# OnurBasci/TransformerBasedNavierStokeSolver

Hardware: AMD Instinct MI355X
Metric: ns64_train_samples_per_s (higher is better)
Workload: dtype f32

## Files before the change

### transformerbasednavierstokesolver_amd/csrc/pa2d_conv_halo.hip

```cpp
#include "pa2d_gemm_common.h"

namespace {
constexpr int TH = 8, TW = 32, BM = TH * TW, BN = 128;
constexpr int HH = TH + 2, HWD = TW + 2, HROWS = HH * HWD;
}

template <int NT, typename TO = float, int TPB = (NT == 1 ? 3 : 1), bool MF16 = false>
__global__ __launch_bounds__(512, 1) void conv_halo_kernel(const KCParams p, const int tiles_x, const int tiles_y,
                                                           const int nimg) {
    constexpr int PITCHB = NT * 64 + (MF16 ? 32 : 16);
    constexpr int PIECES = NT * 4;
    constexpr int A_BYTES = HROWS * PITCHB;
    constexpr int B_TAP = BN * PITCHB;
    constexpr int B_STAGE = TPB * B_TAP;
    constexpr int SPC = 9 / TPB;
    constexpr int AP_IT = (HROWS * PIECES + 255) / 256;
    constexpr int BP_IT = (TPB * BN * PIECES) / 256;
    constexpr int TM = 4, TN = 2;
    static_assert(9 % TPB == 0, "taps per stage");
    extern __shared__ __attribute__((aligned(16))) unsigned char smem[];
    unsigned char* const a_s = smem;
    unsigned char* const b_s = smem + A_BYTES;

    const int tid = threadIdx.x, lane = tid & 63, wave = tid >> 6;
    const int tiles_n = (p.N + BN - 1) / BN;
    const int tiles_m = nimg * tiles_y * tiles_x;
    const int tmx = (tiles_m + 7) / 8;
    const int xcd = blockIdx.x & 7, slot = blockIdx.x >> 3;
    const int tile_m = xcd * tmx + slot / tiles_n;
    const int tile_n = slot % tiles_n;
    if (tile_m >= tiles_m || slot / tiles_n >= tmx) return;
    const int img = tile_m / (tiles_y * tiles_x);
    const int trem = tile_m - img * (tiles_y * tiles_x);
    const int y0 = (trem / tiles_x) * TH, x0 = (trem % tiles_x) * TW;
    const int nch = p.Cin / 32;
    const int nk = nch * 9;
    const int nst = nch * SPC;

    if (wave >= 4) {
        const int ptid = tid - 256;
        const __amdgpu_buffer_rsrc_t ra_rsrc = make_rsrc(p.A, p.a_bytes);
        const __amdgpu_buffer_rsrc_t rb_rsrc = make_rsrc(p.B, p.b_bytes);
        unsigned ap_off[AP_IT], ap_lds[AP_IT];
#pragma unroll
        for (int s = 0; s < AP_IT; ++s) {
            const int q = ptid + 256 * s, row = q / PIECES, piece = q - row * PIECES;
            const int hy = row / HWD, hx = row - hy * HWD;
            const int yy = y0 - 1 + hy, xx = x0 - 1 + hx;
            const bool ok = row < HROWS && (unsigned)yy < (unsigned)p.H && (unsigned)xx < (unsigned)p.W;
            ap_off[s] = ok ? ((unsigned)((img * p.H + yy) * p.W + xx) * (unsigned)(nch * PIECES) + piece) * 16u : OOB_OFF;
            ap_lds[s] = row < HROWS ? (unsigned)(row * PITCHB + piece * 16) : 0xFFFFFFFFu;
        }
        unsigned bp_off[BP_IT], bp_lds[BP_IT];
#pragma unroll
        for (int s = 0; s < BP_IT; ++s) {
            const int q = ptid + 256 * s, tapi = q / (BN * PIECES), r = q - tapi * (BN * PIECES);
            const int row = r / PIECES, piece = r - row * PIECES;
            const int gn = tile_n * BN + row;
            bp_off[s] = gn < p.N ? ((unsigned)gn * (unsigned)nk * PIECES + (unsigned)(tapi * PIECES) + piece) * 16u : OOB_OFF;
            bp_lds[s] = tapi * B_TAP + row * PITCHB + piece * 16;
        }
        u32x4 rq[AP_IT], rp0[BP_IT], rp1[BP_IT];
#define HA_LOAD(chunk_)                                                                                    \
    {                                                                                                      \
        const unsigned sh_ = (unsigned)(chunk_) * (PIECES * 16u);                                          \
        _Pragma("unroll") for (int s = 0; s < AP_IT; ++s)                                                  \
            rq[s] = __builtin_amdgcn_raw_buffer_load_b128(ra_rsrc, ap_off[s] != OOB_OFF ? ap_off[s] + sh_ : OOB_OFF, 0, 0); \
    }
#define HA_STORE()                                                                                         \
    {                                                                                                      \
        _Pragma("unroll") for (int s = 0; s < AP_IT; ++s)                                                  \
            if (ap_lds[s] != 0xFFFFFFFFu) *reinterpret_cast<u32x4*>(a_s + ap_lds[s]) = rq[s];              \
    }
#define HB_LOAD(sg_, RP)                       \
    {                                                                                                      \
        _Pragma("unroll") for (int s = 0; s < BP_IT; ++s)                                                  \
            RP[s] = __builtin_amdgcn_raw_buffer_load_b128(                                                 \
                rb_rsrc, bp_off[s] != OOB_OFF ? bp_off[s] + (unsigned)((sg_) * TPB) * (PIECES * 16u) : OOB_OFF, 0, 0); \
    }
#define HB_STORE(stage_, RP)                                                                               \
    {                                                                                                      \
        _Pragma("unroll") for (int s = 0; s < BP_IT; ++s)                                                  \
            *reinterpret_cast<u32x4*>(b_s + (stage_) * B_STAGE + bp_lds[s]) = RP[s];                       \
    }
#define HB_STEP(sg_, RP_NEXT)                      \
    {                                                                                                      \
        if ((sg_) + 1 < nst) {                                                                             \
            HB_STORE(((sg_) + 1) & 1, RP_NEXT)                                                             \
            if ((sg_) + 5 < nst) HB_LOAD((sg_) + 5, RP_NEXT)                                               \
        }                                                                                                  \
        __syncthreads();                                                              \
        if ((sg_) % SPC == SPC - 1 && (sg_) + 1 < nst) {   \
            HA_STORE()                                                                                     \
            if ((sg_) / SPC + 2 < nch) HA_LOAD((sg_) / SPC + 2)                                            \
            __syncthreads();                                                                               \
        }                                                                                                  \
    }
        u32x4 rp2[BP_IT], rp3[BP_IT];
        HA_LOAD(0)
        HB_LOAD(0, rp0)
        if (nst > 1) HB_LOAD(1, rp1)
        if (nst > 2) HB_LOAD(2, rp2)
        if (nst > 3) HB_LOAD(3, rp3)
        HA_STORE()
        HB_STORE(0, rp0)
        if (nch > 1) HA_LOAD(1)
        if (nst > 4) HB_LOAD(4, rp0)
        __syncthreads();
        for (int sg = 0; sg < nst; sg += 4) {
            HB_STEP(sg, rp1)
            if (sg + 1 < nst) HB_STEP(sg + 1, rp2)
            if (sg + 2 < nst) HB_STEP(sg + 2, rp3)
            if (sg + 3 < nst) HB_STEP(sg + 3, rp0)
        }
#undef HB_STEP
#undef HA_LOAD
#undef HA_STORE
#undef HB_LOAD
#undef HB_STORE
        return;
    }

    const int wm = wave >> 1, wn = wave & 1;
    if constexpr (MF16) {
        static_assert(NT == 3 && TPB == 1, "the 16x16x32 consumers are written for the split engine");
        const int li = lane & 15, kq = lane >> 4;
        f32x4 acc[8][4];
#pragma unroll
        for (int ib = 0; ib < 8; ++ib)
#pragma unroll
            for (int j = 0; j < 4; ++j) acc[ib][j] = f32x4{0.f, 0.f, 0.f, 0.f};
        const unsigned a_frag = (unsigned)((((wm * 4 + 1) * HWD) + 1 + li) * PITCHB + kq * 16);
        const unsigned b_frag = (unsigned)((wn * 64 + li) * PITCHB + kq * 16);
        __syncthreads();
        int tap = 0;
        for (int sg = 0; sg < nst; ++sg) {
            const int dy = tap / 3 - 1, dx = tap - (tap / 3) * 3 - 1;
            const unsigned char* af_base = a_s + a_frag + (dy * HWD + dx) * PITCHB;
            const unsigned char* bf_base = b_s + (sg & 1) * B_STAGE + b_frag;
            bf16x8 bf[4][NT];
#pragma unroll
            for (int j = 0; j < 4; ++j)
#pragma unroll
                for (int q = 0; q < NT; ++q) bf[j][q] = *reinterpret_cast<const bf16x8*>(bf_base + j * 16 * PITCHB + q * 64);
#pragma unroll
            for (int ib = 0; ib < 8; ++ib) {
                bf16x8 af[NT];
#pragma unroll
                for (int q = 0; q < NT; ++q)
                    af[q] = *reinterpret_cast<const bf16x8*>(af_base + (ib >> 1) * (HWD * PITCHB) + (ib & 1) * 16 * PITCHB + q * 64);
#pragma unroll
                for (int j = 0; j < 4; ++j) {
                    acc[ib][j] = __builtin_amdgcn_mfma_f32_16x16x32_bf16(bf[j][1], af[1], acc[ib][j], 0, 0, 0);
                    acc[ib][j] = __builtin_amdgcn_mfma_f32_16x16x32_bf16(bf[j][0], af[2], acc[ib][j], 0, 0, 0);
                    acc[ib][j] = __builtin_amdgcn_mfma_f32_16x16x32_bf16(bf[j][2], af[0], acc[ib][j], 0, 0, 0);
                    acc[ib][j] = __builtin_amdgcn_mfma_f32_16x16x32_bf16(bf[j][0], af[1], acc[ib][j], 0, 0, 0);
                    acc[ib][j] = __builtin_amdgcn_mfma_f32_16x16x32_bf16(bf[j][1], af[0], acc[ib][j], 0, 0, 0);
                    acc[ib][j] = __builtin_amdgcn_mfma_f32_16x16x32_bf16(bf[j][0], af[0], acc[ib][j], 0, 0, 0);
                }
            }
            ++tap;
            __syncthreads();
            if (tap == 9) {
                tap = 0;
                if (sg + 1 < nst) __syncthreads();
            }
        }
        const __amdgpu_buffer_rsrc_t rc = make_rsrc(p.C, p.c_bytes);
        constexpr unsigned ES = Act<TO>::ES;
        const unsigned ldc_b = (unsigned)p.ldc * ES, roww_b = (unsigned)p.W * ldc_b;
        const bool inside = y0 + TH <= p.H && x0 + TW <= p.W;
#pragma unroll
        for (int j = 0; j < 4; ++j) {
            const int col = tile_n * BN + wn * 64 + j * 16 + 4 * kq;
            const bool col_ok = col < p.N;
            float bv[4];
#pragma unroll
            for (int e = 0; e < 4; ++e)
                bv[e] = (p.bias && col_ok) ? (col + e < p.bias_split ? p.bias[col + e] : p.bias2[col + e - p.bias_split]) : 0.f;
#pragma unroll
            for (int ib = 0; ib < 8; ++ib) {
                const int y = y0 + wm * 4 + (ib >> 1), x = x0 + (ib & 1) * 16 + li;
                const bool ok = col_ok && (inside || (y < p.H && x < p.W));
                const unsigned off = ok ? (unsigned)((img * p.H + y) * p.W + x) * ldc_b + (unsigned)col * ES : OOB_OFF;
                float v[4];
#pragma unroll
                for (int e = 0; e < 4; ++e) v[e] = acc[ib][j][e] + bv[e];
                if constexpr (ES == 4) {
                    const u32x4 u = {__float_as_uint(v[0]), __float_as_uint(v[1]), __float_as_uint(v[2]), __float_as_uint(v[3])};
                    __builtin_amdgcn_raw_buffer_store_b128(u, rc, off, 0, 0);
                } else {
                    typedef unsigned int u32x2_ __attribute__((ext_vector_type(2)));
                    const u32x2_ u = {(unsigned)f32_to_bf16_bits(v[0]) | ((unsigned)f32_to_bf16_bits(v[1]) << 16),
                                      (unsigned)f32_to_bf16_bits(v[2]) | ((unsigned)f32_to_bf16_bits(v[3]) << 16)};
                    __builtin_amdgcn_raw_buffer_store_b64(u, rc, off, 0, 0);
                }
            }
        }
        (void)roww_b;
        return;
    }
    f32x16 acc[TM][TN];
#pragma unroll
    for (int i = 0; i < TM; ++i)
#pragma unroll
        for (int j = 0; j < TN; ++j)
#pragma unroll
            for (int r = 0; r < 16; ++r) acc[i][j][r] = 0.f;
    const unsigned a_frag = (unsigned)((((wm * 4 + 1) * HWD) + 1 + (lane & 31)) * PITCHB + (lane >> 5) * 16);
    const unsigned b_frag = (unsigned)((wn * 64 + (lane & 31)) * PITCHB + (lane >> 5) * 16);
    __syncthreads();
    int tap = 0;
    for (int sg = 0; sg < nst; ++sg) {
#pragma unroll
        for (int tt = 0; tt < TPB; ++tt, ++tap) {
            const int dy = tap / 3 - 1, dx = tap - (tap / 3) * 3 - 1;
            const unsigned char* af_base = a_s + a_frag + (dy * HWD + dx) * PITCHB;
            const unsigned char* bf_base = b_s + (sg & 1) * B_STAGE + tt * B_TAP + b_frag;
#pragma unroll
            for (int ks = 0; ks < 2; ++ks) {
                bf16x8 af[TM][NT], bf[TN][NT];
#pragma unroll
                for (int i = 0; i < TM; ++i)
#pragma unroll
                    for (int q = 0; q < NT; ++q)
                        af[i][q] = *reinterpret_cast<const bf16x8*>(af_base + i * (HWD * PITCHB) + q * 64 + ks * 32);
#pragma unroll
                for (int j = 0; j < TN; ++j)
#pragma unroll
                    for (int q = 0; q < NT; ++q)
                        bf[j][q] = *reinterpret_cast<const bf16x8*>(bf_base + j * 32 * PITCHB + q * 64 + ks * 32);
#pragma unroll
                for (int i = 0; i < TM; ++i)
#pragma unroll
                    for (int j = 0; j < TN; ++j) {
                        if constexpr (NT == 3) {
                            acc[i][j] = __builtin_amdgcn_mfma_f32_32x32x16_bf16(af[i][1], bf[j][1], acc[i][j], 0, 0, 0);
                            acc[i][j] = __builtin_amdgcn_mfma_f32_32x32x16_bf16(af[i][2], bf[j][0], acc[i][j], 0, 0, 0);
                            acc[i][j] = __builtin_amdgcn_mfma_f32_32x32x16_bf16(af[i][0], bf[j][2], acc[i][j], 0, 0, 0);
                            acc[i][j] = __builtin_amdgcn_mfma_f32_32x32x16_bf16(af[i][1], bf[j][0], acc[i][j], 0, 0, 0);
                            acc[i][j] = __builtin_amdgcn_mfma_f32_32x32x16_bf16(af[i][0], bf[j][1], acc[i][j], 0, 0, 0);
                        }
                        acc[i][j] = __builtin_amdgcn_mfma_f32_32x32x16_bf16(af[i][0], bf[j][0], acc[i][j], 0, 0, 0);
                    }
            }
        }
        __syncthreads();
        if (tap == 9) {
            tap = 0;
            if (sg + 1 < nst) __syncthreads();
        }
    }

    const __amdgpu_buffer_rsrc_t rc = make_rsrc(p.C, p.c_bytes);
    constexpr unsigned ES = Act<TO>::ES;
    if (y0 + TH <= p.H && x0 + TW <= p.W) {
        const unsigned ldc_b = (unsigned)p.ldc * ES, roww_b = (unsigned)p.W * ldc_b;
#pragma unroll
        for (int j = 0; j < TN; ++j) {
            const int col = tile_n * BN + wn * 64 + j * 32 + (lane & 31);
            const bool col_ok = col < p.N;
            const float bv = (p.bias && col_ok) ? (col < p.bias_split ? p.bias[col] : p.bias2[col - p.bias_split]) : 0.f;
            const unsigned vo = col_ok ? (unsigned)((img * p.H + y0 + wm * 4) * p.W + x0 + 4 * (lane >> 5)) * ldc_b + (unsigned)col * ES
                                       : OOB_OFF;
#pragma unroll
            for (int i = 0; i < TM; ++i)
#pragma unroll
                for (int r = 0; r < 16; ++r) {
                    const unsigned so = (unsigned)i * roww_b + (unsigned)((r & 3) + 8 * (r >> 2)) * ldc_b;
                    if constexpr (ES == 4) __builtin_amdgcn_raw_buffer_store_b32(__float_as_uint(acc[i][j][r] + bv), rc, vo, so, 0);
                    else __builtin_amdgcn_raw_buffer_store_b16(f32_to_bf16_bits(acc[i][j][r] + bv), rc, vo, so, 0);
                }
        }
        return;
    }
#pragma unroll
    for (int j = 0; j < TN; ++j) {
        const int col = tile_n * BN + wn * 64 + j * 32 + (lane & 31);
        const bool col_ok = col < p.N;
        const float bv = (p.bias && col_ok) ? (col < p.bias_split ? p.bias[col] : p.bias2[col - p.bias_split]) : 0.f;
#pragma unroll
        for (int i = 0; i < TM; ++i) {
            const int y = y0 + wm * 4 + i;
            const unsigned rowbase = (unsigned)((img * p.H + y) * p.W);
#pragma unroll
            for (int r = 0; r < 16; ++r) {
                const int x = x0 + 4 * (lane >> 5) + (r & 3) + 8 * (r >> 2);
                const bool ok = col_ok && y < p.H && x < p.W;
                Act<TO>::bst1(rc, ok ? ((rowbase + (unsigned)x) * (unsigned)p.ldc + (unsigned)col) * ES : OOB_OFF,
                              acc[i][j][r] + bv);
            }
        }
    }
}

static int halo_policy() { return pa2d_env().conv_halo; }

bool conv_halo_applies(const KCParams& p) {
    const int pol = halo_policy();
    if (p.taps == 27) return false;
    if (pol == 0 || !p.apre || (p.Cin % 32) != 0 || p.H <= 0 || p.W <= 0 || (p.M % (p.H * p.W)) != 0) return false;
    const long long tiles = (long long)(p.M / (p.H * p.W)) * ceil_div(p.H, TH) * ceil_div(p.W, TW) * ceil_div(p.N, BN);
    return pol == 2 || tiles >= 512;
}

int launch_conv_halo(const KCParams& p, hipStream_t st) {
    const int NT = p.engine == 2 ? 1 : 3;
    const int tiles_x = ceil_div(p.W, TW), tiles_y = ceil_div(p.H, TH), nimg = p.M / (p.H * p.W);
    const int tiles_m = nimg * tiles_y * tiles_x, tiles_n = ceil_div(p.N, BN);
    const dim3 grid(ceil_div(tiles_m, 8) * 8 * tiles_n);
    const int pitch = NT * 64 + 16;
    const int smem = HROWS * pitch + 2 * (NT == 1 ? 3 : 1) * BN * pitch;
    if (NT == 3 && pa2d_env().conv_mfma16 && (p.N % 4) == 0 && (p.ldc % 4) == 0) {
        const int smem16 = (HROWS + 2 * BN) * (3 * 64 + 32);
        {
            hipError_t e = hipFuncSetAttribute(reinterpret_cast<const void*>(&conv_halo_kernel<3, float, 1, true>),
                                               hipFuncAttributeMaxDynamicSharedMemorySize, smem16);
            if (e != hipSuccess) return (int)e;
        }
        hipLaunchKernelGGL((conv_halo_kernel<3, float, 1, true>), grid, dim3(512), smem16, st, p, tiles_x, tiles_y, nimg);
    } else if (NT == 3) {
        {
            hipError_t e = hipFuncSetAttribute(reinterpret_cast<const void*>(&conv_halo_kernel<3>),
                                               hipFuncAttributeMaxDynamicSharedMemorySize, smem);
            if (e != hipSuccess) return (int)e;
        }
        hipLaunchKernelGGL((conv_halo_kernel<3>), grid, dim3(512), smem, st, p, tiles_x, tiles_y, nimg);
    } else if (p.io_bf16) {
        {
            hipError_t e = hipFuncSetAttribute(reinterpret_cast<const void*>(&conv_halo_kernel<1, bf16_t>),
                                               hipFuncAttributeMaxDynamicSharedMemorySize, smem);
            if (e != hipSuccess) return (int)e;
        }
        hipLaunchKernelGGL((conv_halo_kernel<1, bf16_t>), grid, dim3(512), smem, st, p, tiles_x, tiles_y, nimg);
    } else {
        {
            hipError_t e = hipFuncSetAttribute(reinterpret_cast<const void*>(&conv_halo_kernel<1>),
                                               hipFuncAttributeMaxDynamicSharedMemorySize, smem);
            if (e != hipSuccess) return (int)e;
        }
        hipLaunchKernelGGL((conv_halo_kernel<1>), grid, dim3(512), smem, st, p, tiles_x, tiles_y, nimg);
    }
    PA2D_CHECK_LAUNCH();
    return PA2D_OK;
}
```

### transformerbasednavierstokesolver_amd/csrc/pa2d_gemm.hip

```cpp
#include "pa2d_gemm_common.h"
#include <string.h>


static Pa2dEnv read_env() {
    auto is = [](const char* n, const char* pre) { const char* e = getenv(n); return e && strncmp(e, pre, strlen(pre)) == 0; };
    auto num = [](const char* n, int dflt) { const char* e = getenv(n); return (e && e[0]) ? atoi(e) : dflt; };
    Pa2dEnv v;
    v.conv_halo = is("PA2D_CONV_HALO", "o") ? 0 : (is("PA2D_CONV_HALO", "f") ? 2 : 1);
    v.mc_big_off = is("PA2D_MC_BIG", "o") ? 1 : 0;
    v.kc_bk16 = num("PA2D_KC_BK", 0) == 16 ? 1 : 0;
    v.mc_bk = num("PA2D_MC_BK", 16) == 32 ? 32 : 16;
    v.mc_splits = num("PA2D_MC_SPLITS", 0);
    v.mcb_splits = num("PA2D_MCB_SPLITS", 0);
    v.lin_dw_split = is("PA2D_LIN_DW_SPLIT", "of") ? 0 : 1;
    v.lin_panel = is("PA2D_LIN_PANEL", "of") ? 0 : 1;
    v.lin_rowpanel = is("PA2D_LIN_ROWPANEL", "of") ? 0 : 1;
    v.lin_small_split = is("PA2D_LIN_SMALL_SPLIT", "of") ? 0 : 1;
    v.conv_mfma16 = num("PA2D_CONV_MFMA", 16) == 32 ? 0 : 1;
    v.mc_mfma16 = num("PA2D_MC_MFMA", 16) == 32 ? 0 : 1;
    v.split_big = num("PA2D_SPLIT_BIG", 1);
    v.slice_map = is("PA2D_SLICE_MAP", "l") ? 0 : 1;
    v.default_engine = is("PA2D_GEMM", "f") ? 0 : (is("PA2D_GEMM", "b") ? 2 : 1);
    return v;
}
static Pa2dEnv g_env = read_env();
const Pa2dEnv& pa2d_env() { return g_env; }
static int kc_bk(bool im2col, int Cin) {
    if (im2col && pa2d_env().kc_bk16) return 16;
    return (!im2col || (Cin % 32) == 0) ? 32 : 16;
}
KCTile kc_tile(int M, int N, bool im2col, int Cin) {
    const int tiles_m = ceil_div(M, 128);
    const long long t128 = (long long)tiles_m * ceil_div(N, 128);
    const long long t12864 = (long long)tiles_m * ceil_div(N, 64);
    const int bk = kc_bk(im2col, Cin);
    if (N > 64 && t128 >= 384) return {128, 128, bk};
    if (t12864 >= 384 || M <= 64) return {128, 64, bk};
    return {64, 64, bk};
}
bool use_split(int engine, int N, bool im2col, int Cin) {
    const int m = engine;
    if (m == 1) return im2col && N > 64 && (Cin % 32) == 0;
    if (m == 2) return N > 64 && (!im2col || (Cin % 32) == 0);
    return false;
}

int launch_kc(const KCParams& p_in, bool im2col, hipStream_t st, hipEvent_t ev0, hipEvent_t ev1) {
    KCParams p = p_in;
    if (!engine_ok(p.engine)) return PA2D_ERR_ARG;
    if (p.M <= 0 || p.N <= 0 || p.K <= 0) return PA2D_OK;
    if (!p.bias2) p.bias_split = 0x7fffffff;
    {
        const unsigned long long ab = ((unsigned long long)(p.M - 1) * p.lda + (im2col ? p.Cin : p.K)) * 4ull;
        const unsigned long long bb = ((unsigned long long)(p.N - 1) * p.ldb + p.K) * 4ull;
        if (ab >= 0xFFFFFFF0ull || bb >= 0xFFFFFFF0ull) return PA2D_ERR_UNSUPPORTED;
        p.a_bytes = (unsigned)ab;
        p.b_bytes = (unsigned)bb;
        const unsigned long long es = p.io_bf16 ? 2ull : 4ull;
        const unsigned long long cb = ((unsigned long long)(p.M - 1) * p.ldc + p.N) * es;
        const unsigned long long rb = p.res ? ((unsigned long long)(p.M - 1) * p.ldres + p.N) * es : 0ull;
        const unsigned long long xb = p.aux ? ((unsigned long long)(p.M - 1) * p.ldaux + p.N) * es : 0ull;
        if (cb >= 0xFFFFFFF0ull || rb >= 0xFFFFFFF0ull || xb >= 0xFFFFFFF0ull) return PA2D_ERR_UNSUPPORTED;
        p.c_bytes = (unsigned)cb; p.res_bytes = (unsigned)rb; p.aux_bytes = (unsigned)xb;
    }
    if ((p.K & 3) || (p.lda & 3) || (p.ldb & 3)) return PA2D_ERR_ARG;
    if (im2col && ((p.Cin & 15) || p.K != (p.taps == 27 ? 27 : 9) * p.Cin)) return PA2D_ERR_UNSUPPORTED;
    if (im2col && (p.epi != 0 || p.res)) return PA2D_ERR_ARG;
    if (ev0 && hipEventRecord(ev0, st) != hipSuccess) return PA2D_ERR_ARG;
    int rc;
    if (!im2col && p.wimg && rowpanel_applies(p)) {
        if (p.wsrc) {
            rc = launch_pack_weight_image(p.wsrc, p.wsn, p.wsk, p.wimg, p.N, p.K, st);
            if (rc) return rc;
        }
        KCParams pp = p;
        pp.M = p.M - p.M % 128;
        rc = launch_kc_rowpanel(pp, p.wimg, st);
        if (!rc && pp.M < p.M) {
            KCParams pt = p_in;
            pt.wimg = nullptr;
            pt.M = p.M - pp.M;
            pt.A = p.A + (size_t)pp.M * p.lda;
            pt.C = p.C + (size_t)pp.M * p.ldc;
            if (p.res) pt.res = p.res + (size_t)pp.M * p.ldres;
            if (p.aux) pt.aux = p.aux + (size_t)pp.M * p.ldaux;
            rc = launch_kc(pt, false, st);
        }
    } else if (panel_applies(p, im2col)) {
        KCParams pp = p;
        pp.M = p.M - p.M % 256;
        rc = launch_kc_panel(pp, st);
        if (!rc && pp.M < p.M) {
            KCParams pt = p_in;
            const size_t ea = p.io_bf16 ? 2 : 4, es = p.io_bf16 ? 2 : 4;
            pt.M = p.M - pp.M;
            pt.A = (const float*)((const char*)p.A + (size_t)pp.M * p.lda * ea);
            pt.C = (float*)((char*)p.C + (size_t)pp.M * p.ldc * es);
            if (p.res) pt.res = (const float*)((const char*)p.res + (size_t)pp.M * p.ldres * es);
            if (p.aux) pt.aux = (float*)((char*)p.aux + (size_t)pp.M * p.ldaux * es);
            rc = launch_kc(pt, false, st);
        }
    } else if (p.io_bf16 || use_split(p.engine, p.N, im2col, p.Cin)) rc = launch_kc_split(p, im2col, st);
    else if (kc_split_small_applies(p, im2col)) rc = launch_kc_split_small(p, st);
    else rc = launch_kc_f32(p, im2col, kc_tile(p.M, p.N, im2col, p.Cin), st);
    if (rc) return rc;
    if (ev1 && hipEventRecord(ev1, st) != hipSuccess) return PA2D_ERR_ARG;
    return PA2D_OK;
}

template <int TAPS>
__global__ void repack_kernel(const float* __restrict__ w0, const float* __restrict__ w1, float* __restrict__ dst,
                              int mode, int N, int K, int C, int Cin, int NK) {
    const long long idx = (long long)blockIdx.x * blockDim.x + threadIdx.x;
    if (mode == 0) {
        if (idx >= (long long)N * K) return;
        const int n = (int)(idx % N), k = (int)(idx / N);
        dst[idx] = w0[(size_t)n * K + k];
    } else if (mode == 1) {
        if (idx >= (long long)NK * C * TAPS * Cin) return;
        const int CH = K;
        const int c16 = (int)(idx % CH);
        const int tap = (int)((idx / CH) % TAPS);
        const int cic = (int)((idx / (TAPS * CH)) % (Cin / CH));
        const int co = (int)(idx / ((long long)Cin * TAPS));
        const int ci = cic * CH + c16;
        const float* src = co < C ? w0 : w1;
        dst[idx] = src[((size_t)(co % C) * Cin + ci) * TAPS + tap];
    } else {
        if (idx >= (long long)NK * C * TAPS * Cin) return;
        const int CH = K;
        const int c16 = (int)(idx % CH);
        const int tap = (int)((idx / CH) % TAPS);
        const int cic = (int)((idx / (TAPS * CH)) % (NK * C / CH));
        const int ci = (int)(idx / ((long long)NK * C * TAPS));
        const int co = cic * CH + c16;
        const float* src = co < C ? w0 : w1;
        dst[idx] = src[((size_t)(co % C) * Cin + ci) * TAPS + (TAPS - 1 - tap)];
    }
}

int launch_repack(const float* w0, const float* w1, float* dst, int mode, int N, int K, int C, int Cin, hipStream_t st,
                  int taps) {
    const int nk = w1 ? 2 : 1;
    const long long count = mode == 0 ? (long long)N * K : (long long)nk * C * taps * Cin;
    const dim3 grid((unsigned)ceil_div_ll(count, 256));
    if (taps == 27)
        hipLaunchKernelGGL(repack_kernel<27>, grid, dim3(256), 0, st, w0, w1, dst, mode, N, K, C, Cin, nk);
    else
        hipLaunchKernelGGL(repack_kernel<9>, grid, dim3(256), 0, st, w0, w1, dst, mode, N, K, C, Cin, nk);
    PA2D_CHECK_LAUNCH();
    return PA2D_OK;
}

static KCParams dense_fwd_params(const void* x, long long ldx, const float* w, long long ldw, const float* bias,
                                 const void* res, long long ldres, void* y, long long ldy, void* pre, long long ldpre, int M,
                                 int N, int K, int act, int engine, bool io_bf16) {
    KCParams p = {};
    p.engine = engine; p.io_bf16 = io_bf16 ? 1 : 0; p.apre = io_bf16 ? 1 : 0;
    p.aux_deriv = (act & PA2D_ACT_SAVE_DERIVATIVE_BIT) ? 1 : 0;
    act &= ~PA2D_ACT_SAVE_DERIVATIVE_BIT;
    p.A = (const float*)x; p.lda = ldx; p.B = w; p.ldb = ldw; p.C = (float*)y; p.ldc = ldy; p.bias = bias;
    p.res = (const float*)res; p.ldres = ldres; p.aux = (float*)pre; p.ldaux = ldpre; p.M = M; p.N = N; p.K = K; p.act = act;
    p.epi = (act != ACT_NONE ? EPI_ACT : 0) | (pre ? EPI_STORE_PRE : 0);
    return p;
}
static KCParams dense_bwd_data_params(const void* dy, long long lddy, const float* wt, const void* pre, long long ldpre,
                                      int act, void* dx, long long lddx, int M, int N, int K, int engine, bool io_bf16) {
    KCParams p = {};
    p.engine = engine; p.io_bf16 = io_bf16 ? 1 : 0; p.apre = io_bf16 ? 1 : 0;
    p.aux_deriv = (act & PA2D_ACT_SAVE_DERIVATIVE_BIT) ? 1 : 0;
    act &= ~PA2D_ACT_SAVE_DERIVATIVE_BIT;
// ... 129 lines not shown
```

### transformerbasednavierstokesolver_amd/csrc/pa2d_gemm_rowpanel.hip

```cpp
#include "pa2d_gemm_common.h"
#include <type_traits>
#ifndef RP_SGB
#define RP_SGB 1
#endif

namespace {

constexpr int RP_STAGE = 24 * 1024;
constexpr int RP_SLOTS = 3;
constexpr int RP_BIAS = 4096;

typedef unsigned int u32x4_ __attribute__((ext_vector_type(4)));

__device__ __forceinline__ float4 ld4s(__amdgpu_buffer_rsrc_t r, unsigned voff, unsigned soff) {
    const u32x4_ v = __builtin_amdgcn_raw_buffer_load_b128(r, voff, soff, 0);
    return make_float4(__uint_as_float(v.x), __uint_as_float(v.y), __uint_as_float(v.z), __uint_as_float(v.w));
}
__device__ __forceinline__ void st4s(__amdgpu_buffer_rsrc_t r, unsigned voff, unsigned soff, const float (&v)[4]) {
    const u32x4_ u = {__float_as_uint(v[0]), __float_as_uint(v[1]), __float_as_uint(v[2]), __float_as_uint(v[3])};
    __builtin_amdgcn_raw_buffer_store_b128(u, r, voff, soff, 0);
}
__device__ __forceinline__ bf16x8 cat8(bf16x4 a, bf16x4 b) { return __builtin_shufflevector(a, b, 0, 1, 2, 3, 4, 5, 6, 7); }

__global__ void pack_weight_image_kernel(const float* __restrict__ src, long long sn, long long sk, unsigned char* __restrict__ img,
// ... 15 lines not shown
    *reinterpret_cast<bf16x8*>(dst + 1024) = cat8(m0, m1);
    *reinterpret_cast<bf16x8*>(dst + 2048) = cat8(l0, l1);
}

template <int KS, int MODE, bool HAS_RES>
__global__ __launch_bounds__(256, 1) void gemm_rowpanel_kernel(const KCParams p, const unsigned char* __restrict__ img,
                                                               const unsigned img_bytes) {
    constexpr int KC = KS / 4;
    extern __shared__ __attribute__((aligned(16))) unsigned char smem[];
    const int tid = threadIdx.x, lane = tid & 63;
    const int wave = __builtin_amdgcn_readfirstlane(tid >> 6);
    const int li = lane & 15, kq = lane >> 4;
    const int NP = p.N / 64, SPR = NP * KC;
    float* const bias_s = reinterpret_cast<float*>(smem);
    unsigned char* const ring = smem + RP_BIAS;
    for (int c = tid; c < p.N; c += 256)
        bias_s[c] = (MODE != 2 && p.bias) ? (c < p.bias_split ? p.bias[c] : p.bias2[c - p.bias_split]) : 0.f;
    const int rounds = p.M / 128;
    const int n_my = ((int)blockIdx.x < rounds) ? (rounds - (int)blockIdx.x + (int)gridDim.x - 1) / (int)gridDim.x : 0;
    if (n_my == 0) return;
    const int T = n_my * SPR;

    const __amdgpu_buffer_rsrc_t ra = make_rsrc(p.A, p.a_bytes);
    const __amdgpu_buffer_rsrc_t ri = make_rsrc_v(img, img_bytes);
    const __amdgpu_buffer_rsrc_t rc = make_rsrc(p.C, p.c_bytes);
    const __amdgpu_buffer_rsrc_t rres = make_rsrc(p.res ? p.res : p.C, p.res ? p.res_bytes : 0u);
    const __amdgpu_buffer_rsrc_t raux = make_rsrc(p.aux ? p.aux : p.C, p.aux ? p.aux_bytes : 0u);
    const unsigned lda_b = (unsigned)p.lda * 4u, ldc_b = (unsigned)p.ldc * 4u, ldres_b = (unsigned)p.ldres * 4u,
                   ldaux_b = (unsigned)p.ldaux * 4u;

    const unsigned piece = (unsigned)(wave * 6) * 1024u + (unsigned)lane * 16u;
    u32x4_ breg[6];
    int ld_stage = 0;
    auto stage_load = [&]() {
#pragma unroll
        for (int i = 0; i < 6; ++i)
            breg[i] = __builtin_amdgcn_raw_buffer_load_b128(ri, piece + i * 1024u, (unsigned)ld_stage * RP_STAGE, 0);
        if (++ld_stage == SPR) ld_stage = 0;
    };
    auto stage_write = [&](int slot) {
#pragma unroll
        for (int i = 0; i < 6; ++i) *reinterpret_cast<u32x4_*>(ring + slot * RP_STAGE + piece + i * 1024) = breg[i];
    };

    const unsigned a_voff = (unsigned)li * lda_b + (unsigned)kq * 32u;
    float4 raw[KS][2];
    bf16x8 ap[KS][3];
    auto a_load = [&](int u, unsigned voff, unsigned row0) {
        const unsigned so = (row0 + 16u * (u & 1)) * lda_b;
        raw[u][0] = ld4s(ra, voff == OOB_OFF ? OOB_OFF : voff + (u >> 1) * 128u, so);
        raw[u][1] = ld4s(ra, voff == OOB_OFF ? OOB_OFF : voff + (u >> 1) * 128u + 16u, so);
    };
    auto a_split = [&](int ks) {
        bf16x4 h0, m0, l0, h1, m1, l1;
        split3(raw[ks][0], h0, m0, l0);
        split3(raw[ks][1], h1, m1, l1);
        ap[ks][0] = cat8(h0, h1); ap[ks][1] = cat8(m0, m1); ap[ks][2] = cat8(l0, l1);
    };

    int round = blockIdx.x;
    unsigned row0 = (unsigned)(round * 128 + wave * 32);
#pragma unroll
    for (int ks = 0; ks < KS; ++ks) a_load(ks, a_voff, row0);
    stage_load();
    stage_write(0);
    stage_load();
#pragma unroll
    for (int ks = 0; ks < KS; ++ks) a_split(ks);
    __syncthreads();

    const unsigned vc = li * ldc_b + kq * 16u, vr = li * ldres_b + kq * 16u, vx = li * ldaux_b + kq * 16u;

    bf16x8 bfb[2][2][3];
    int cur = 0;
    auto frag_read = [&](int buf, int slot, int ks4) {
        const unsigned char* bs = ring + slot * RP_STAGE + lane * 16;
#pragma unroll
        for (int j = 0; j < 2; ++j)
#pragma unroll
            for (int u = 0; u < 3; ++u) bfb[buf][j][u] = *reinterpret_cast<const bf16x8*>(bs + ((ks4 * 2 + j) * 3 + u) * 1024);
    };
    frag_read(0, 0, 0);

    f32x4 acc[2][4];
    float4 ov[2][4];
    auto ep_group = [&](const int q8, const int np) {
        const int rb = q8 >> 2, nt = q8 & 3;
        const unsigned cb = (unsigned)(np * 64 + nt * 16) * 4u;
        const unsigned rw = row0 + 16u * rb;
        float v[4];
#pragma unroll
        for (int e = 0; e < 4; ++e) v[e] = acc[rb][nt][e];
        if (MODE == 1) {
            if (p.aux_deriv) {
                float d[4];
#pragma unroll
                for (int e = 0; e < 4; ++e) d[e] = dgelu_f(v[e]);
                st4s(raux, vx, rw * ldaux_b + cb, d);
            } else {
                st4s(raux, vx, rw * ldaux_b + cb, v);
            }
#pragma unroll
            for (int e = 0; e < 4; ++e) v[e] = gelu_f(v[e]);
        } else if (MODE == 2) {
            if (p.aux_deriv) {
                v[0] *= ov[rb][nt].x; v[1] *= ov[rb][nt].y; v[2] *= ov[rb][nt].z; v[3] *= ov[rb][nt].w;
            } else {
                v[0] *= dgelu_f(ov[rb][nt].x); v[1] *= dgelu_f(ov[rb][nt].y); v[2] *= dgelu_f(ov[rb][nt].z); v[3] *= dgelu_f(ov[rb][nt].w);
            }
        } else if (HAS_RES) {
            v[0] += ov[rb][nt].x; v[1] += ov[rb][nt].y; v[2] += ov[rb][nt].z; v[3] += ov[rb][nt].w;
        }
#ifdef RP_NO_STORE
        if (p.M == 12345)
#endif
        st4s(rc, vc, rw * ldc_b + cb, v);
    };
    auto ov_load = [&](const int q8, const int np) {
        const int rb = q8 >> 2, nt = q8 & 3;
        const unsigned cb = (unsigned)(np * 64 + nt * 16) * 4u;
        if (MODE == 2) ov[rb][nt] = ld4s(raux, vx, (row0 + 16u * rb) * ldaux_b + cb);
        else if (HAS_RES) ov[rb][nt] = ld4s(rres, vr, (row0 + 16u * rb) * ldres_b + cb);
    };

    unsigned row0n = 0, a_voff_n = OOB_OFF;
    auto pair = [&](auto first_tag, auto last_tag, const int np) {
        constexpr bool FIRST = decltype(first_tag)::value, LAST = decltype(last_tag)::value;
#pragma unroll
        for (int nt = 0; nt < 4; ++nt) {
            const float4 bv = *reinterpret_cast<const float4*>(bias_s + np * 64 + nt * 16 + 4 * kq);
#pragma unroll
            for (int rb = 0; rb < 2; ++rb) {
                acc[rb][nt] = f32x4{bv.x, bv.y, bv.z, bv.w};
                ov_load(rb * 4 + nt, np);
            }
        }
#pragma unroll
        for (int kc = 0; kc < KC; ++kc) {
            const int nxt = cur == 2 ? 0 : cur + 1;
#ifndef RP_NO_BSTAGE
            stage_write(nxt);
            stage_load();
#endif
#ifndef RP_NO_ANEXT
            if (FIRST) {
#pragma unroll
                for (int q = 0; q < 4; ++q) a_load(kc * 4 + q, a_voff_n, row0n);
            }
#endif
#pragma unroll
            for (int ks4 = 0; ks4 < 4; ++ks4) {
                if (ks4 < 3) frag_read((ks4 + 1) & 1, cur, ks4 + 1);
                else frag_read(0, nxt, 0);
                const int ks = kc * 4 + ks4;
#ifndef RP_NO_ANEXT
                if (LAST && kc >= 1) a_split(ks - 4);
                if (FIRST && kc == 0) a_split(KS - 4 + ks4);
#endif
#define RP_MFMA(u_, v_)                                                                                      \
    _Pragma("unroll") for (int j = 0; j < 2; ++j) _Pragma("unroll") for (int rb = 0; rb < 2; ++rb)            \
        acc[rb][2 * (ks4 & 1) + j] = __builtin_amdgcn_mfma_f32_16x16x32_bf16(                                 \
            bfb[ks4 & 1][j][v_], ap[kc * 4 + (ks4 >> 1) * 2 + rb][u_], acc[rb][2 * (ks4 & 1) + j], 0, 0, 0);
#ifndef RP_NO_MFMA
                RP_MFMA(1, 1) RP_MFMA(2, 0) RP_MFMA(0, 2) RP_MFMA(1, 0) RP_MFMA(0, 1) RP_MFMA(0, 0)
#endif
#undef RP_MFMA
#if RP_SGB == 1
#pragma unroll
                for (int i = 0; i < 6; ++i) {
                    __builtin_amdgcn_sched_group_barrier(0x008, 4, 0);
                    __builtin_amdgcn_sched_group_barrier(0x100, 1, 0);
                }
#endif
#ifndef RP_NO_BARRIER
                if (ks4 == 1) __syncthreads();
#endif
            }
            cur = nxt;
        }
#pragma unroll
        for (int q8 = 0; q8 < 8; ++q8) ep_group(q8, np);
    };
    using T_ = std::true_type; using F_ = std::false_type;

    for (int t = 0; t < n_my; ++t) {
        const bool more = t + 1 < n_my;
        row0n = more ? (unsigned)((round + (int)gridDim.x) * 128 + wave * 32) : 0u;
        a_voff_n = more ? a_voff : OOB_OFF;
        pair(T_{}, F_{}, 0);
        for (int np = 1; np < NP - 1; ++np) pair(F_{}, F_{}, np);
        pair(F_{}, T_{}, NP - 1);
        round += gridDim.x;
        row0 = row0n;
    }
}

template <int KS, int MODE, bool HAS_RES>
int launch_rowpanel_t(const KCParams& p, const unsigned char* img, hipStream_t st) {
    const int smem = RP_BIAS + RP_SLOTS * RP_STAGE;
    {
        hipError_t e = hipFuncSetAttribute(reinterpret_cast<const void*>(&gemm_rowpanel_kernel<KS, MODE, HAS_RES>),
                                           hipFuncAttributeMaxDynamicSharedMemorySize, smem);
        if (e != hipSuccess) return (int)e;
    }
    const int rounds = p.M / 128;
    const unsigned img_bytes = (unsigned)((size_t)p.N * p.K * 6);
    hipLaunchKernelGGL((gemm_rowpanel_kernel<KS, MODE, HAS_RES>), dim3(rounds < 256 ? rounds : 256), dim3(256), smem, st, p,
                       img, img_bytes);
    PA2D_CHECK_LAUNCH();
    return PA2D_OK;
}

int rowpanel_mode(const KCParams& p) {
    const bool gelu = p.act == ACT_GELU, has_res = p.res != nullptr;
    if (p.epi == 0) return 0;
    if (gelu && !has_res && (p.epi == (EPI_ACT | EPI_STORE_PRE) || p.epi == EPI_ACT)) return 1;
    if (gelu && !has_res && p.epi == EPI_MUL_DACT && !p.bias) return 2;
    return -1;
}

template <int KS>
int launch_rowpanel_k(const KCParams& p, const unsigned char* img, hipStream_t st) {
    switch (rowpanel_mode(p)) {
        case 0: return p.res ? launch_rowpanel_t<KS, 0, true>(p, img, st) : launch_rowpanel_t<KS, 0, false>(p, img, st);
        case 1: return launch_rowpanel_t<KS, 1, false>(p, img, st);
        case 2: return launch_rowpanel_t<KS, 2, false>(p, img, st);
        default: return PA2D_ERR_ARG;
    }
}

}

size_t rowpanel_image_bytes(int N, int K, int engine) {
    if (engine != 1 || (K != 128 && K != 256) || N < 128 || N > 1024 || (N % 128) != 0) return 0;
    return (size_t)N * K * 6;
}

bool rowpanel_applies(const KCParams& p) {
    if (!pa2d_env().lin_rowpanel || p.io_bf16) return false;
    if (rowpanel_image_bytes(p.N, p.K, p.engine) == 0) return false;
    if (rowpanel_mode(p) < 0 || (p.epi == EPI_ACT && p.aux)) return false;
    if ((p.lda & 3) || (p.ldc & 3) || (p.res && (p.ldres & 3)) || (p.aux && (p.ldaux & 3))) return false;
    return p.M / 128 >= 256;
}

int launch_pack_weight_image(const float* w, long long sn, long long sk, void* img, int N, int K, hipStream_t st) {
    const int count = (N / 64) * (K / 64) * 8 * 64;
    hipLaunchKernelGGL(pack_weight_image_kernel, dim3(ceil_div(count, 256)), dim3(256), 0, st, w, sn, sk, (unsigned char*)img, N, K);
    PA2D_CHECK_LAUNCH();
    return PA2D_OK;
}

int launch_kc_rowpanel(const KCParams& p, const void* img, hipStream_t st) {
    if (p.K == 256) return launch_rowpanel_k<16>(p, (const unsigned char*)img, st);
    return launch_rowpanel_k<8>(p, (const unsigned char*)img, st);
}
```

### transformerbasednavierstokesolver_amd/csrc/pa2d_internal.h

```cpp
#pragma once
#include <hip/hip_runtime.h>
#include <stdint.h>

typedef float f32x16 __attribute__((ext_vector_type(16)));
typedef float f32x4 __attribute__((ext_vector_type(4)));

#define PA2D_OK 0
#define PA2D_ERR_ARG 1001
#define PA2D_ERR_UNSUPPORTED 1002
#define PA2D_ERR_WORKSPACE 1003

#define PA2D_CHECK_LAUNCH()                         \
    do {                                            \
        hipError_t e__ = hipGetLastError();         \
        if (e__ != hipSuccess) return (int)e__;     \
    } while (0)

enum { ACT_NONE = 0, ACT_GELU = 1, ACT_TANH = 2, ACT_SIGMOID = 3, ACT_RELU = 4, ACT_SOFTPLUS = 5,
       ACT_ELU = 6, ACT_SILU = 7 };

__device__ __forceinline__ float normal_cdf(float x, float& e_out) {
#pragma clang fp contract(off)
    const float z = fabsf(x) * 0.70710678118654752440f;
    const float t = __builtin_amdgcn_rcpf(fmaf(0.3275911f, z, 1.0f));
    float poly = fmaf(1.061405429f, t, -1.453152027f);
    poly = fmaf(poly, t, 1.421413741f);
    poly = fmaf(poly, t, -0.284496736f);
    poly = fmaf(poly, t, 0.254829592f);
    const float e = __builtin_amdgcn_exp2f(-z * z * 1.44269504088896340736f);
    e_out = e;
    const float hq = 0.5f * poly * t * e;
    return x < 0.f ? hq : 1.0f - hq;
}
__device__ __forceinline__ float gelu_exact(float x) {
#pragma clang fp contract(off)
    float e;
    return x * normal_cdf(x, e);
}
__device__ __forceinline__ float dgelu_exact(float x) {
#pragma clang fp contract(off)
    float e;
    const float cdf = normal_cdf(x, e);
    return fmaf(x * 0.39894228040143267794f, e, cdf);
}

__device__ __forceinline__ float act_fwd(int id, float x) {
    switch (id) {
        case ACT_GELU: return gelu_exact(x);
        case ACT_TANH: return tanhf(x);
        case ACT_SIGMOID: return 1.0f / (1.0f + expf(-x));
        case ACT_RELU: return x > 0.f ? x : 0.f;
        case ACT_SOFTPLUS: return x > 20.f ? x : log1pf(expf(x));
        case ACT_ELU: return x > 0.f ? x : expm1f(x);
        case ACT_SILU: return x / (1.0f + expf(-x));
        default: return x;
    }
}

__device__ __forceinline__ float act_bwd(int id, float x) {
    switch (id) {
        case ACT_GELU: return dgelu_exact(x);
        case ACT_TANH: { const float t = tanhf(x); return 1.0f - t * t; }
        case ACT_SIGMOID: { const float s = 1.0f / (1.0f + expf(-x)); return s * (1.0f - s); }
        case ACT_RELU: return x > 0.f ? 1.f : 0.f;
        case ACT_SOFTPLUS: return x > 20.f ? 1.f : 1.0f / (1.0f + expf(-x));
        case ACT_ELU: return x > 0.f ? 1.f : expf(x);
        case ACT_SILU: { const float s = 1.0f / (1.0f + expf(-x)); return s * (1.0f + x * (1.0f - s)); }
        default: return 1.f;
    }
}

__device__ __forceinline__ float wave_sum(float v) {
#pragma unroll
    for (int o = 32; o > 0; o >>= 1) v += __shfl_xor(v, o, 64);
    return v;
}
__device__ __forceinline__ float wave_max(float v) {
#pragma unroll
    for (int o = 32; o > 0; o >>= 1) v = fmaxf(v, __shfl_xor(v, o, 64));
    return v;
}

typedef unsigned int u32x4 __attribute__((ext_vector_type(4)));
#define OOB_OFF 0xFFFFFFFFu

__device__ __forceinline__ __amdgpu_buffer_rsrc_t make_rsrc(const float* base, unsigned bytes) {
    return __builtin_amdgcn_make_buffer_rsrc(const_cast<float*>(base), 0, bytes, 0x00020000);
}
__device__ __forceinline__ float4 buf_load4(__amdgpu_buffer_rsrc_t r, unsigned voff) {
    const u32x4 v = __builtin_amdgcn_raw_buffer_load_b128(r, voff, 0, 0);
    return make_float4(__uint_as_float(v.x), __uint_as_float(v.y), __uint_as_float(v.z), __uint_as_float(v.w));
}


__device__ __forceinline__ float buf_load1(__amdgpu_buffer_rsrc_t r, unsigned voff) {
    return __uint_as_float(__builtin_amdgcn_raw_buffer_load_b32(r, voff, 0, 0));
}
__device__ __forceinline__ void buf_store1(__amdgpu_buffer_rsrc_t r, unsigned voff, float v) {
    __builtin_amdgcn_raw_buffer_store_b32(__float_as_uint(v), r, voff, 0, 0);
}

__device__ __forceinline__ float2 buf_load2(__amdgpu_buffer_rsrc_t r, unsigned voff) {
    typedef unsigned int u32x2_ __attribute__((ext_vector_type(2)));
    const u32x2_ v = __builtin_amdgcn_raw_buffer_load_b64(r, voff, 0, 0);
    return make_float2(__uint_as_float(v.x), __uint_as_float(v.y));
}
__device__ __forceinline__ void buf_store4(__amdgpu_buffer_rsrc_t r, unsigned voff, float4 v) {
    u32x4 u = {__float_as_uint(v.x), __float_as_uint(v.y), __float_as_uint(v.z), __float_as_uint(v.w)};
    __builtin_amdgcn_raw_buffer_store_b128(u, r, voff, 0, 0);
}

#define PA2D_ACT_SAVE_DERIVATIVE_BIT 0x100

struct Pa2dEnv {
    int conv_halo;
    int mc_big_off;
    int kc_bk16;
    int mc_bk;
    int mc_splits;
    int mcb_splits;
    int lin_dw_split;
    int lin_panel;
    int conv_mfma16;
    int mc_mfma16;
    int lin_small_split;
    int lin_rowpanel;
    int split_big;
    int slice_map;
    int default_engine;
};
const Pa2dEnv& pa2d_env();

static inline int pa2d_zero(void* p, size_t bytes, hipStream_t st) {
    if (!p || !bytes) return PA2D_OK;
    return (int)hipMemsetAsync(p, 0, bytes, st);
}
static inline int ceil_div(int a, int b) { return (a + b - 1) / b; }
static inline long long ceil_div_ll(long long a, long long b) { return (a + b - 1) / b; }

struct ReduceSegs { int nseg; long long begin[5]; float* dst[4]; };
int pa2d_launch_reduce_segs(const float* slab, int nslab, long long count, const ReduceSegs& segs, int accumulate,
                            hipStream_t st);

typedef __bf16 bf16_t;
template <typename T> struct Act;
template <> struct Act<float> {
    static constexpr unsigned ES = 4;
    static __device__ __forceinline__ float4 ld4(const float* p) { return *reinterpret_cast<const float4*>(p); }
    static __device__ __forceinline__ void st4(float* p, float4 v) { *reinterpret_cast<float4*>(p) = v; }
    static __device__ __forceinline__ float ld1(const float* p) { return *p; }
    static __device__ __forceinline__ float4 bld4(__amdgpu_buffer_rsrc_t r, unsigned off) { return buf_load4(r, off); }
    static __device__ __forceinline__ float2 bld2(__amdgpu_buffer_rsrc_t r, unsigned off) { return buf_load2(r, off); }
    static __device__ __forceinline__ float bld1(__amdgpu_buffer_rsrc_t r, unsigned off) { return buf_load1(r, off); }
    static __device__ __forceinline__ float bld1s(__amdgpu_buffer_rsrc_t r, unsigned off, unsigned soff) {
        return __uint_as_float(__builtin_amdgcn_raw_buffer_load_b32(r, off, soff, 0));
    }
    static __device__ __forceinline__ void bst4(__amdgpu_buffer_rsrc_t r, unsigned off, float4 v) { buf_store4(r, off, v); }
    static __device__ __forceinline__ void bst1(__amdgpu_buffer_rsrc_t r, unsigned off, float v) { buf_store1(r, off, v); }
};
__device__ __forceinline__ float bf16_bits_to_f32(unsigned short b) { return __uint_as_float((unsigned)b << 16); }
__device__ __forceinline__ unsigned short f32_to_bf16_bits(float x) {
    const bf16_t h = (bf16_t)x;
    return __builtin_bit_cast(unsigned short, h);
}
__device__ __forceinline__ unsigned pack_bf16x2(float lo, float hi) {
    return (unsigned)f32_to_bf16_bits(lo) | ((unsigned)f32_to_bf16_bits(hi) << 16);
}
template <> struct Act<bf16_t> {
    static constexpr unsigned ES = 2;
    static __device__ __forceinline__ float4 unpack4(uint2 q) {
        return make_float4(__uint_as_float(q.x << 16), __uint_as_float(q.x & 0xFFFF0000u), __uint_as_float(q.y << 16),
                           __uint_as_float(q.y & 0xFFFF0000u));
    }
    static __device__ __forceinline__ float4 ld4(const bf16_t* p) { return unpack4(*reinterpret_cast<const uint2*>(p)); }
    static __device__ __forceinline__ void st4(bf16_t* p, float4 v) {
        *reinterpret_cast<uint2*>(p) = make_uint2(pack_bf16x2(v.x, v.y), pack_bf16x2(v.z, v.w));
    }
    static __device__ __forceinline__ float ld1(const bf16_t* p) { return (float)*p; }
    static __device__ __forceinline__ float4 bld4(__amdgpu_buffer_rsrc_t r, unsigned off) {
        typedef unsigned int u32x2_ __attribute__((ext_vector_type(2)));
        const u32x2_ q = __builtin_amdgcn_raw_buffer_load_b64(r, off, 0, 0);
        return unpack4(make_uint2(q.x, q.y));
    }
    static __device__ __forceinline__ float2 bld2(__amdgpu_buffer_rsrc_t r, unsigned off) {
        const unsigned q = __builtin_amdgcn_raw_buffer_load_b32(r, off, 0, 0);
        return make_float2(__uint_as_float(q << 16), __uint_as_float(q & 0xFFFF0000u));
    }
    static __device__ __forceinline__ float bld1(__amdgpu_buffer_rsrc_t r, unsigned off) {
        return bf16_bits_to_f32(__builtin_amdgcn_raw_buffer_load_b16(r, off, 0, 0));
    }
    static __device__ __forceinline__ float bld1s(__amdgpu_buffer_rsrc_t r, unsigned off, unsigned soff) {
        return bf16_bits_to_f32(__builtin_amdgcn_raw_buffer_load_b16(r, off, soff, 0));
    }
    static __device__ __forceinline__ void bst4(__amdgpu_buffer_rsrc_t r, unsigned off, float4 v) {
        typedef unsigned int u32x2_ __attribute__((ext_vector_type(2)));
        const u32x2_ q = {pack_bf16x2(v.x, v.y), pack_bf16x2(v.z, v.w)};
        __builtin_amdgcn_raw_buffer_store_b64(q, r, off, 0, 0);
    }
    static __device__ __forceinline__ void bst1(__amdgpu_buffer_rsrc_t r, unsigned off, float v) {
        __builtin_amdgcn_raw_buffer_store_b16(f32_to_bf16_bits(v), r, off, 0, 0);
    }
};
__device__ __forceinline__ __amdgpu_buffer_rsrc_t make_rsrc_v(const void* base, unsigned bytes) {
    return __builtin_amdgcn_make_buffer_rsrc(const_cast<void*>(base), 0, bytes, 0x00020000);
}

__device__ __forceinline__ bool slice_decode(int xcd_map, int B, int heads, int nchunk, int& b, int& hh, int& chunk, int& bid) {
    const int total = B * heads * nchunk;
    int L;
    if (xcd_map) {
        const int per = (total + 7) >> 3;
        if ((int)(blockIdx.x >> 3) >= per) return false;
        L = (int)(blockIdx.x & 7) * per + (int)(blockIdx.x >> 3);
        if (L >= total) return false;
        hh = L % heads;
        chunk = (L / heads) % nchunk;
        b = L / (heads * nchunk);
    } else {
        L = (int)blockIdx.x;
        if (L >= total) return false;
        chunk = L % nchunk;
        hh = (L / nchunk) % heads;
        b = L / (nchunk * heads);
    }
    bid = (b * heads + hh) * nchunk + chunk;
    return true;
}
static inline int slice_grid(int total) { return ((total + 7) / 8) * 8; }
```

Before: 71.66.

## Software-pipeline LDS fragment loads ahead of MFMAs in halo conv kernel

```diff
diff --git a/transformerbasednavierstokesolver_amd/csrc/pa2d_conv_halo.hip b/transformerbasednavierstokesolver_amd/csrc/pa2d_conv_halo.hip
--- a/transformerbasednavierstokesolver_amd/csrc/pa2d_conv_halo.hip
+++ b/transformerbasednavierstokesolver_amd/csrc/pa2d_conv_halo.hip
@@ -5,9 +5,8 @@
 constexpr int HH = TH + 2, HWD = TW + 2, HROWS = HH * HWD;
 }
 
-template <int NT, typename TO = float, int TPB = (NT == 1 ? 3 : 1), bool MF16 = false>
-__global__ __launch_bounds__(512, 1) void conv_halo_kernel(const KCParams p, const int tiles_x, const int tiles_y,
-                                                           const int nimg) {
+template <int NT, typename TO, int TPB, bool MF16, bool AHEAD>
+__device__ __forceinline__ void conv_halo_body(const KCParams& p, const int tiles_x, const int tiles_y, const int nimg) {
     constexpr int PITCHB = NT * 64 + (MF16 ? 32 : 16);
     constexpr int PIECES = NT * 4;
     constexpr int A_BYTES = HROWS * PITCHB;
@@ -134,6 +133,68 @@
         const unsigned b_frag = (unsigned)((wn * 64 + li) * PITCHB + kq * 16);
         __syncthreads();
         int tap = 0;
+        if constexpr (AHEAD) {
+            bf16x8 bf[4][NT], a0[NT], a1[NT];
+#define CH_PIN() __builtin_amdgcn_sched_barrier(0)
+#define CH_LDA(AF_, base_, ib_)                                                                            \
+    {                                                                                                      \
+        _Pragma("unroll") for (int q = 0; q < NT; ++q)                                                     \
+            AF_[q] = *reinterpret_cast<const bf16x8*>((base_) + ((ib_) >> 1) * (HWD * PITCHB) + ((ib_) & 1) * 16 * PITCHB + q * 64); \
+        CH_PIN();                                                                                          \
+    }
+#define CH_LDB(j_, base_)                                                                                  \
+    {                                                                                                      \
+        _Pragma("unroll") for (int q = 0; q < NT; ++q)                                                     \
+            bf[j_][q] = *reinterpret_cast<const bf16x8*>((base_) + (j_) * 16 * PITCHB + q * 64);          \
+        CH_PIN();                                                                                          \
+    }
+#define CH_T(ib_, j_, AF_, bq_, aq_) \
+    acc[ib_][j_] = __builtin_amdgcn_mfma_f32_16x16x32_bf16(bf[j_][bq_], AF_[aq_], acc[ib_][j_], 0, 0, 0);
+#define CH_MM(ib_, j_, AF_)               \
+    {                                                                                                      \
+        CH_T(ib_, j_, AF_, 1, 1) CH_T(ib_, j_, AF_, 0, 2) CH_T(ib_, j_, AF_, 2, 0)                         \
+        CH_T(ib_, j_, AF_, 0, 1) CH_T(ib_, j_, AF_, 1, 0) CH_T(ib_, j_, AF_, 0, 0)                         \
+        CH_PIN();                                                                                          \
+    }
+#define CH_BLOCK(ib_, AF_) CH_MM(ib_, 0, AF_) CH_MM(ib_, 1, AF_) CH_MM(ib_, 2, AF_) CH_MM(ib_, 3, AF_)
+            const unsigned char* af_base = a_s + a_frag + (-HWD - 1) * PITCHB;
+            const unsigned char* bf_base = b_s + b_frag;
+            CH_PIN();
+            CH_LDB(0, bf_base) CH_LDB(1, bf_base) CH_LDA(a0, af_base, 0) CH_LDB(2, bf_base) CH_LDB(3, bf_base)
+            for (int sg = 0; sg < nst; ++sg) {
+                const bool swap = tap == 8;
+                const int ntap = swap ? 0 : tap + 1;
+                const int ndy = ntap / 3 - 1, ndx = ntap - (ntap / 3) * 3 - 1;
+                const unsigned char* af_next = a_s + a_frag + (ndy * HWD + ndx) * PITCHB;
+                const unsigned char* bf_next = b_s + ((sg + 1) & 1) * B_STAGE + b_frag;
+                CH_PIN();
+                CH_LDA(a1, af_base, 1) CH_BLOCK(0, a0)
+                CH_LDA(a0, af_base, 2) CH_BLOCK(1, a1)
+                CH_LDA(a1, af_base, 3) CH_BLOCK(2, a0)
+                CH_LDA(a0, af_base, 4) CH_BLOCK(3, a1)
+                CH_LDA(a1, af_base, 5) CH_BLOCK(4, a0)
+                CH_LDA(a0, af_base, 6) CH_BLOCK(5, a1)
+                CH_LDA(a1, af_base, 7) CH_MM(6, 0, a0) CH_MM(6, 1, a0)
+                __syncthreads();
+                CH_PIN();
+                CH_MM(7, 0, a1) CH_LDB(0, bf_next)
+                CH_MM(7, 1, a1) CH_LDB(1, bf_next)
+                CH_MM(6, 2, a0) CH_MM(6, 3, a0)
+                if (swap && sg + 1 < nst) __syncthreads();
+                CH_PIN();
+                CH_LDA(a0, af_next, 0)
+                CH_MM(7, 2, a1) CH_LDB(2, bf_next)
+                CH_MM(7, 3, a1) CH_LDB(3, bf_next)
+                af_base = af_next;
+                tap = ntap;
+            }
+#undef CH_BLOCK
+#undef CH_MM
+#undef CH_T
+#undef CH_LDB
+#undef CH_LDA
+#undef CH_PIN
+        } else
         for (int sg = 0; sg < nst; ++sg) {
             const int dy = tap / 3 - 1, dx = tap - (tap / 3) * 3 - 1;
             const unsigned char* af_base = a_s + a_frag + (dy * HWD + dx) * PITCHB;
@@ -294,6 +355,16 @@
     }
 }
 
+template <int NT, typename TO = float, int TPB = (NT == 1 ? 3 : 1), bool MF16 = false>
+__global__ __launch_bounds__(512, 1) void conv_halo_kernel(const KCParams p, const int tiles_x, const int tiles_y,
+                                                           const int nimg) {
+    conv_halo_body<NT, TO, TPB, MF16, MF16>(p, tiles_x, tiles_y, nimg);
+}
+__global__ __launch_bounds__(512, 1) void conv_halo_ref_kernel(const KCParams p, const int tiles_x, const int tiles_y,
+                                                               const int nimg) {
+    conv_halo_body<3, float, 1, true, false>(p, tiles_x, tiles_y, nimg);
+}
+
 static int halo_policy() { return pa2d_env().conv_halo; }
 
 bool conv_halo_applies(const KCParams& p) {
@@ -313,12 +384,13 @@
     const int smem = HROWS * pitch + 2 * (NT == 1 ? 3 : 1) * BN * pitch;
     if (NT == 3 && pa2d_env().conv_mfma16 && (p.N % 4) == 0 && (p.ldc % 4) == 0) {
         const int smem16 = (HROWS + 2 * BN) * (3 * 64 + 32);
+        auto* const kern = pa2d_env().conv_ahead ? &conv_halo_kernel<3, float, 1, true> : &conv_halo_ref_kernel;
         {
-            hipError_t e = hipFuncSetAttribute(reinterpret_cast<const void*>(&conv_halo_kernel<3, float, 1, true>),
+            hipError_t e = hipFuncSetAttribute(reinterpret_cast<const void*>(kern),
                                                hipFuncAttributeMaxDynamicSharedMemorySize, smem16);
             if (e != hipSuccess) return (int)e;
         }
-        hipLaunchKernelGGL((conv_halo_kernel<3, float, 1, true>), grid, dim3(512), smem16, st, p, tiles_x, tiles_y, nimg);
+        hipLaunchKernelGGL(kern, grid, dim3(512), smem16, st, p, tiles_x, tiles_y, nimg);
     } else if (NT == 3) {
         {
             hipError_t e = hipFuncSetAttribute(reinterpret_cast<const void*>(&conv_halo_kernel<3>),
diff --git a/transformerbasednavierstokesolver_amd/csrc/pa2d_gemm.hip b/transformerbasednavierstokesolver_amd/csrc/pa2d_gemm.hip
--- a/transformerbasednavierstokesolver_amd/csrc/pa2d_gemm.hip
+++ b/transformerbasednavierstokesolver_amd/csrc/pa2d_gemm.hip
@@ -17,6 +17,7 @@
     v.lin_rowpanel = is("PA2D_LIN_ROWPANEL", "of") ? 0 : 1;
     v.lin_small_split = is("PA2D_LIN_SMALL_SPLIT", "of") ? 0 : 1;
     v.conv_mfma16 = num("PA2D_CONV_MFMA", 16) == 32 ? 0 : 1;
+    v.conv_ahead = num("PA2D_CONV_AHEAD", 1) == 0 ? 0 : 1;
     v.mc_mfma16 = num("PA2D_MC_MFMA", 16) == 32 ? 0 : 1;
     v.split_big = num("PA2D_SPLIT_BIG", 1);
     v.slice_map = is("PA2D_SLICE_MAP", "l") ? 0 : 1;
diff --git a/transformerbasednavierstokesolver_amd/csrc/pa2d_gemm_rowpanel.hip b/transformerbasednavierstokesolver_amd/csrc/pa2d_gemm_rowpanel.hip
--- a/transformerbasednavierstokesolver_amd/csrc/pa2d_gemm_rowpanel.hip
+++ b/transformerbasednavierstokesolver_amd/csrc/pa2d_gemm_rowpanel.hip
@@ -191,6 +191,9 @@
             for (int ks4 = 0; ks4 < 4; ++ks4) {
                 if (ks4 < 3) frag_read((ks4 + 1) & 1, cur, ks4 + 1);
                 else frag_read(0, nxt, 0);
+#if RP_SGB == 2
+                __builtin_amdgcn_sched_barrier(0);
+#endif
                 const int ks = kc * 4 + ks4;
 #ifndef RP_NO_ANEXT
                 if (LAST && kc >= 1) a_split(ks - 4);
diff --git a/transformerbasednavierstokesolver_amd/csrc/pa2d_internal.h b/transformerbasednavierstokesolver_amd/csrc/pa2d_internal.h
--- a/transformerbasednavierstokesolver_amd/csrc/pa2d_internal.h
+++ b/transformerbasednavierstokesolver_amd/csrc/pa2d_internal.h
@@ -122,6 +122,7 @@
     int lin_dw_split;
     int lin_panel;
     int conv_mfma16;
+    int conv_ahead;
     int mc_mfma16;
     int lin_small_split;
     int lin_rowpanel;
```

New measurement: 74.02 (median of 6 runs). +3.3%, better.
